# marcopesavento/Super-resolution-3D-Human-Shape-from-a-Single-Low-Resolution-Image

Hardware: AMD Instinct MI355X
Metric: occupancy queries/sec (dense 512^3 reconstruction: encoder + query sweep + 2x marching cubes) (higher is better)
Workload: dtype bf16

## Files before the change

### super-resolution-3d-human-shape-from-a-single-low-resolution-image_amd/csrc/surs_api.cpp

```cpp
#include "surs_common.h"

extern "C" int surs_abi_version(void) { return SURS_ABI_VERSION; }

extern "C" const char *surs_last_error(void) { return surs::err_buf(); }

extern "C" int surs_device_info(int *cu_count, char *arch_out) {
    int dev = 0;
    SURS_HIP_CHECK(hipGetDevice(&dev));
    hipDeviceProp_t prop;
    SURS_HIP_CHECK(hipGetDeviceProperties(&prop, dev));
    if (cu_count) *cu_count = prop.multiProcessorCount;
    if (arch_out) {
        strncpy(arch_out, prop.gcnArchName, 31);
        arch_out[31] = 0;
    }
    return 0;
}

#include <atomic>
#include <cstdlib>
#include <mutex>

namespace {
struct OptionRow {
    const char *name, *env;
    int def;
    char env_first;
    int env_value;
    const char *what;
};
const OptionRow kOptions[surs::OPT_COUNT] = {
    {"split_parts", "SURS_SPLIT", 2, 'b', 3, "operand parts of the fp32-grade GEMMs: 2 (f16 x 2) or 3 (bf16 x 3; env: bf16x3)"},
    {"grid_f32_columns", "SURS_GRID_F32", 1, 'g', 0, "0 (env: gemm): the fp32 sweep on the per-point layer kernels"},
    {"grid_kernel", "SURS_GRID_KERNEL", 0, 0, 0, "reduced-precision column kernel: 0 (default 12), 3, 10, 12"},
    {"grid_f32_kernel", "SURS_GRID_F32_KERNEL", 0, 0, 0, "fp32-grade column kernel: 0 (default 11), 5, 11"},
    {"r_parts", "SURS_R_PARTS", 1, 0, 0, "1: the bf16 sweep's R vectors from one f16 part; 0: the sweep's split"},
    {"grid_f32_passes", "SURS_GRID_F32_PASSES", 2, 0, 0, "passes of the fp32-grade column kernel per batch: 2 (lr, then hr) or 1"},
    {"bicubic_block", "SURS_BICUBIC_BLOCK", 1, 0, 0, "0: bicubic x2 with statistics one output per item (A/B; same bits)"},
    {"mc_emit_reclassify", "SURS_MC_EMIT_RECLASSIFY", 0, 0, 0, "1: marching cubes' emit pass classifies again (tests)"},
    {"point_runs_speculate", "SURS_POINT_RUNS_SPECULATE", 1, 0, 0, "0: surs_query_points_columns reads the run count before it launches"},
    {"conv_trace", "SURS_CONV_TRACE", 0, 0, 0, "diagnostic builds (-DSURS_CONV_TRACE): print the 3x3 kernel's phase stamps"},
    {"v3_trace", "SURS_V3_TRACE", 0, 0, 0, "diagnostic builds (-DSURS_V3_TRACE): print the column kernels' stamps"},
    {"conv_tall_min_wg", "SURS_CONV_TALL_MIN_WG", 256, 0, 0, "workgroups from which a stride-1 3x3 convolution takes the 8-row tile instead of 4 rows (0: never; same bits)"},
    {"conv_wide_min_wg", "SURS_CONV_WIDE_MIN_WG", 512, 0, 0, "workgroups (of 64 channels) from which such a launch takes 8 rows x 64 channels (part of the bits: another order of sums; 0: never)"},
    {"mc_ring", "SURS_MC_RING", 258, 0, 0, "planes of marching cubes' edge -> vertex-id ring = layers per chunk of a one-piece extraction + 1 (66: round 5's)"},
    {"rvec_small", "SURS_RVEC_SMALL", 1, 0, 0, "0: the affine part's GEMM of batches of <= 1024 columns on the 256 x 256-tile kernel (A/B; same bits)"},
};
std::atomic<int> g_option[surs::OPT_COUNT];
std::once_flag g_option_once;
void import_environment() {
    for (int i = 0; i < surs::OPT_COUNT; ++i) {
        const OptionRow &r = kOptions[i];
        int v = r.def;
        if (const char *e = getenv(r.env)) {
            if (r.env_first) v = (e[0] == r.env_first) ? r.env_value : r.def;
            else if (e[0]) v = atoi(e);
        }
        g_option[i].store(v, std::memory_order_relaxed);
    }
}
int find_option(const char *name) {
    if (!name) return -1;
    for (int i = 0; i < surs::OPT_COUNT; ++i)
        if (!strcmp(name, kOptions[i].name) || !strcmp(name, kOptions[i].env)) return i;
    return -1;
}
}

int surs::option(surs::Opt id) {
    std::call_once(g_option_once, import_environment);
    return g_option[id].load(std::memory_order_relaxed);
}

extern "C" int surs_set_option(const char *name, int value) {
    const int i = find_option(name);
    SURS_REQUIRE(i >= 0, "unknown option '%s' (surs_option_name(i) lists them)", name ? name : "(null)");
    std::call_once(g_option_once, import_environment);
    g_option[i].store(value, std::memory_order_relaxed);
    return 0;
}

extern "C" int surs_get_option(const char *name, int *value) {
    const int i = find_option(name);
    SURS_REQUIRE(i >= 0 && value, "unknown option '%s'", name ? name : "(null)");
    *value = surs::option((surs::Opt)i);
    return 0;
}

extern "C" const char *surs_option_name(int index) { return (index >= 0 && index < surs::OPT_COUNT) ? kOptions[index].name : nullptr; }
extern "C" const char *surs_option_help(int index) { return (index >= 0 && index < surs::OPT_COUNT) ? kOptions[index].what : nullptr; }
```

### super-resolution-3d-human-shape-from-a-single-low-resolution-image_amd/csrc/surs_common.h

```cpp
#pragma once
#include <hip/hip_runtime.h>

#include <cstdarg>
#include <cstdio>
#include <cstring>

#include "../../include/surs.h"

namespace surs {

inline char *err_buf() {
    static thread_local char buf[512] = "";
    return buf;
}

inline int fail(int code, const char *fmt, ...) {
    va_list ap;
    va_start(ap, fmt);
    vsnprintf(err_buf(), 512, fmt, ap);
    va_end(ap);
    return code;
}

#define SURS_HIP_CHECK(expr)                                                                     \
    do {                                                                                         \
        hipError_t e_ = (expr);                                                                  \
        if (e_ != hipSuccess)                                                                    \
            return surs::fail(SURS_E_HIP, "%s:%d %s -> %s", __FILE__, __LINE__, #expr, hipGetErrorString(e_)); \
    } while (0)

#define SURS_LAUNCH_CHECK() SURS_HIP_CHECK(hipGetLastError())

#define SURS_REQUIRE(cond, ...)                                   \
    do {                                                          \
        if (!(cond)) return surs::fail(SURS_E_INVALID, __VA_ARGS__); \
    } while (0)

#ifndef SURS_ABL_NO_ISA_PINS
#define SURS_ISA_PIN(v) asm volatile("" : "+v"(v))
#else
#define SURS_ISA_PIN(v) do { } while (0)
#endif

enum Opt {
    OPT_SPLIT_PARTS, OPT_GRID_F32_COLUMNS, OPT_GRID_KERNEL, OPT_GRID_F32_KERNEL, OPT_R_PARTS,
    OPT_GRID_F32_PASSES, OPT_BICUBIC_BLOCK, OPT_MC_EMIT_RECLASSIFY, OPT_POINT_RUNS_SPECULATE, OPT_CONV_TRACE,
    OPT_V3_TRACE, OPT_CONV_TALL_MIN_WG, OPT_CONV_WIDE_MIN_WG, OPT_MC_RING, OPT_RVEC_SMALL, OPT_COUNT
};
int option(Opt id);

inline hipStream_t as_stream(void *s) { return reinterpret_cast<hipStream_t>(s); }

constexpr int ceil_div(long long a, long long b) { return (int)((a + b - 1) / b); }

struct DeviceOnce {
    unsigned long long mask = 0;
    bool first() {
        int dev = 0;
        if (hipGetDevice(&dev) != hipSuccess || dev < 0 || dev >= 64) return true;
        const unsigned long long bit = 1ull << dev;
        const unsigned long long old = __atomic_fetch_or(&mask, bit, __ATOMIC_ACQ_REL);
        return !(old & bit);
    }
};
inline size_t align_up(size_t v, size_t a) { return (v + a - 1) / a * a; }

}
```

### super-resolution-3d-human-shape-from-a-single-low-resolution-image_amd/csrc/surs_gemm.inc

```
__device__ __forceinline__ bool gemm_block_tile(int mblocks, int nblocks, int &mb, int &nb) {
    const unsigned total = (unsigned)mblocks * (unsigned)nblocks, per = gridDim.x >> 3;
    const unsigned logical = (blockIdx.x & 7u) * per + (blockIdx.x >> 3);
    mb = (int)(logical % (unsigned)mblocks);
    nb = (int)(logical / (unsigned)mblocks);
    return logical < total;
}

static inline unsigned gemm_grid(int mblocks, long long nblocks) {
    const long long total = (long long)mblocks * nblocks;
    return (unsigned)(((total + 7) / 8) * 8);
}

struct SplitSeg {
    const unsigned short *base;
    long long part;
    int ktiles;
};

constexpr int G3_STAGES = 3;
constexpr int g3_stage_bytes(int bm, int np_ = 3) { return np_ * ((bm / 32) + 8) * 1024; }
constexpr int g3_lds_bytes(int bm, int np_ = 3) { return G3_STAGES * g3_stage_bytes(bm, np_); }

template <int NP> struct SplitKind;
template <> struct SplitKind<1> {
    typedef _Float16 vec8 __attribute__((ext_vector_type(8)));
    static __device__ __forceinline__ f32x16 mfma(vec8 a, vec8 b, f32x16 c) { return __builtin_amdgcn_mfma_f32_32x32x16_f16(a, b, c, 0, 0, 0); }
    static __device__ __forceinline__ void split(float x, unsigned short (&p)[1]) { p[0] = __builtin_bit_cast(unsigned short, (_Float16)x); }
};
template <> struct SplitKind<3> {
    typedef bf16x8_t vec8;
    static __device__ __forceinline__ f32x16 mfma(vec8 a, vec8 b, f32x16 c) { return __builtin_amdgcn_mfma_f32_32x32x16_bf16(a, b, c, 0, 0, 0); }
    static __device__ __forceinline__ void split(float x, unsigned short (&p)[3]) { split3_bf16(x, p[0], p[1], p[2]); }
};
template <> struct SplitKind<2> {
    typedef _Float16 vec8 __attribute__((ext_vector_type(8)));
    static __device__ __forceinline__ f32x16 mfma(vec8 a, vec8 b, f32x16 c) { return __builtin_amdgcn_mfma_f32_32x32x16_f16(a, b, c, 0, 0, 0); }
    static __device__ __forceinline__ void split(float x, unsigned short (&p)[2]) {
        asm volatile("" : "+v"(x));
        const _Float16 hi = (_Float16)x;
        const _Float16 lo = (_Float16)__builtin_fmaf((float)hi, -1.0f, x);
        p[0] = __builtin_bit_cast(unsigned short, hi);
        p[1] = __builtin_bit_cast(unsigned short, lo);
    }
};

enum { G3_SPLIT = 0, G3_F32 = 1, G3_F32_T = 2 };
template <int NW, int BM, int OUT, int NP = 3>
__global__ __launch_bounds__(NW * 64) void gemm_x3g_kernel(const unsigned short *__restrict__ W3, int M, int Ktot, SplitSeg s1,
                                                           SplitSeg s2, long long np, const float *__restrict__ bias,
                                                           float *__restrict__ Y, long long ldy,
                                                           unsigned short *__restrict__ Ys, long long ys_part, int nblocks) {
    typedef SplitKind<NP> SK;
    typedef typename SK::vec8 vec8;
    constexpr int AP = BM / 32;
    constexpr int TI = AP / 2;
    constexpr int ASZ = NP * AP * 1024;
    constexpr int G3_STAGE = g3_stage_bytes(BM, NP);
    static_assert(NW == 8, "eight waves, 2 x 4");
    static_assert(TI == 4 || TI == 2, "wave tile is 128 or 64 rows");
    static_assert(NP >= 1 && NP <= 3, "one f16 part (not fp32-grade), two f16 parts or three bf16 parts");
    extern __shared__ __attribute__((aligned(16))) unsigned char g3_smem[];
    typedef __attribute__((address_space(3))) unsigned char lds_u8;
    typedef const __attribute__((address_space(1))) void gptr_t;
    const int tid = threadIdx.x, lane = tid & 63, wave = tid >> 6;
    const int wm = wave >> 2, wn = wave & 3;
    const int kh = lane >> 5, li = lane & 31;
    int mb, nb;
    {
        const unsigned mblocks = (unsigned)M / (unsigned)BM, total = mblocks * (unsigned)nblocks, per = gridDim.x >> 3;
        const unsigned logical = (blockIdx.x & 7u) * per + (blockIdx.x >> 3);
        if (logical >= total) return;
        mb = (int)(logical % mblocks);
        nb = (int)(logical / mblocks);
    }
    const long long n0 = (long long)nb * 256;
    const int m0 = mb * BM;
    const int ktiles = s1.ktiles + s2.ktiles;
    const size_t per_part = (size_t)Ktot * M;
    lds_u8 *smem = (lds_u8 *)g3_smem;
    const unsigned lds0 = (unsigned)(size_t)smem;

    f32x16 acc[TI][2];
#pragma unroll
    for (int i = 0; i < TI; ++i)
#pragma unroll
        for (int j = 0; j < 2; ++j)
#pragma unroll
            for (int r = 0; r < 16; ++r) acc[i][j][r] = 0.0f;

    const int piece = wave & 7;
    const bool both = BM == 256 || wave < 4;
    const int nd = both ? 2 * NP : NP;
    const unsigned short *wsrc = W3 + ((size_t)(m0 + 32 * piece)) * 16 + lane * 8;
    auto issue1 = [&](int kt, int d) {
        const int p = both ? d >> 1 : d;
        const bool points = both ? (d & 1) : (NW == 8 || wave >= 8);
        lds_u8 *stage = smem + (kt % G3_STAGES) * G3_STAGE + piece * 1024;
        if (!points) {
            const unsigned short *wk = wsrc + (size_t)kt * M * 16 + p * per_part;
            __builtin_amdgcn_global_load_lds((gptr_t *)wk, (__attribute__((address_space(3))) void *)(stage + p * (AP * 1024)), 16, 0, 0);
        } else {
            const bool first = kt < s1.ktiles;
            const unsigned short *xb = first ? s1.base : s2.base;
            const long long xpart = first ? s1.part : s2.part;
            const int k = first ? kt : kt - s1.ktiles;
            const unsigned short *xsrc = xb + ((long long)k * np + n0 + 32 * piece) * 16 + (li * 16 + kh * 8) + p * xpart;
            __builtin_amdgcn_global_load_lds((gptr_t *)xsrc, (__attribute__((address_space(3))) void *)(stage + ASZ + p * 8192), 16, 0, 0);
        }
    };
    auto issue = [&](int kt) {
        for (int d = 0; d < nd; ++d) issue1(kt, d);
    };

    issue(0);
    if (ktiles > 1) issue(1);
    const unsigned a_off = lds0 + (unsigned)(wm * TI * 1024 + lane * 16);
    const unsigned b_off = lds0 + (unsigned)ASZ + (unsigned)(wn * 2048 + lane * 16);
    vec8 a[TI][NP], b[2][NP];
    auto mm = [&](int pa, int pb) {
#pragma unroll
        for (int i = 0; i < TI; ++i)
#pragma unroll
            for (int j = 0; j < 2; ++j) {
                if constexpr (OUT == G3_F32_T) acc[i][j] = SK::mfma(b[j][pb], a[i][pa], acc[i][j]);
                else acc[i][j] = SK::mfma(a[i][pa], b[j][pb], acc[i][j]);
            }
    };
#ifdef SURS_G3_NO_LDS
#define G3_RD(dst, addr, off) asm volatile("" : "=v"(dst) : "v"(addr) : "memory")
// ... 24 lines not shown
            if constexpr (NP == 3 && TI == 2) { if (t == 0) G3_WAIT2(8, 2, 0); else if (t == 1) G3_WAIT2(4, 1, 1); else G3_WAIT2(0, 0, 2); }
            if constexpr (NP == 2 && TI == 4) { if (t == 0) G3_WAIT4(6, 1, 0); else G3_WAIT4(0, 0, 1); }
            if constexpr (NP == 2 && TI == 2) { if (t == 0) G3_WAIT2(4, 1, 0); else G3_WAIT2(0, 0, 1); }
            if constexpr (NP == 1 && TI == 4) G3_WAIT4(0, 0, 0);
            if constexpr (NP == 1 && TI == 2) G3_WAIT2(0, 0, 0);
            mm(NP - 1 - t, t);
            __builtin_amdgcn_sched_barrier(0);
            if (more)
                for (int d = t * nd / NP; d < (t + 1) * nd / NP; ++d) issue1(kt + 2, d);
        }
    };
    auto phase2 = [&](int kt) {
        if constexpr (NP == 3) {
            mm(1, 0);
            mm(0, 1);
        }
        if constexpr (NP > 1) mm(0, 0);
        __builtin_amdgcn_sched_barrier(0);
    };
    auto step_barrier = [&](int kt) {
#ifdef SURS_G3_NO_DMA
        asm volatile("s_waitcnt vmcnt(0)\n\ts_barrier" ::: "memory");
#else
        if (kt + 1 < ktiles) {
            if (nd == 6) asm volatile("s_waitcnt vmcnt(6)\n\ts_barrier" ::: "memory");
            else if (nd == 4) asm volatile("s_waitcnt vmcnt(4)\n\ts_barrier" ::: "memory");
            else if (nd == 3) asm volatile("s_waitcnt vmcnt(3)\n\ts_barrier" ::: "memory");
            else if (nd == 1) asm volatile("s_waitcnt vmcnt(1)\n\ts_barrier" ::: "memory");
            else asm volatile("s_waitcnt vmcnt(2)\n\ts_barrier" ::: "memory");
        } else
            asm volatile("s_waitcnt vmcnt(0)\n\ts_barrier" ::: "memory");
#endif
    };
    if (((wave >> 2) & 1) == 0) {
        for (int kt = 0; kt < ktiles; ++kt) {
            step_barrier(kt);
            phase1(kt);
            phase2(kt);
        }
    } else {
        step_barrier(0);
        phase1(0);
        for (int kt = 1; kt < ktiles; ++kt) {
            step_barrier(kt);
            phase2(kt - 1);
            phase1(kt);
        }
        phase2(ktiles - 1);
    }

#undef G3_RD
#undef G3_WAIT4
#undef G3_WAIT2
#pragma unroll
    for (int i = 0; i < TI; ++i)
#pragma unroll
        for (int j = 0; j < 2; ++j) {
            const long long n = n0 + wn * 64 + j * 32 + li;
            const int mrow = m0 + wm * (TI * 32) + i * 32;
            if constexpr (OUT == G3_F32_T) {
                const long long nb0 = n0 + wn * 64 + j * 32 + 4 * kh;
                const float bm = bias[mrow + li];
#pragma unroll
                for (int g = 0; g < 4; ++g)
#pragma unroll
                    for (int r = 0; r < 4; ++r) Y[(nb0 + 8 * g + r) * ldy + mrow + li] = acc[i][j][4 * g + r] + bm;
                continue;
            }
            float v[16];
#pragma unroll
            for (int g = 0; g < 4; ++g)
#pragma unroll
                for (int r = 0; r < 4; ++r) {
                    float t = acc[i][j][4 * g + r] + bias[mrow + 8 * g + 4 * kh + r];
                    v[4 * g + r] = t > 0.0f ? t : 0.01f * t;
                }
            if constexpr (OUT == G3_F32) {
#pragma unroll
                for (int g = 0; g < 4; ++g)
#pragma unroll
                    for (int r = 0; r < 4; ++r) Y[(long long)(mrow + 8 * g + 4 * kh + r) * ldy + n] = v[4 * g + r];
            } else
#pragma unroll
            for (int q = 0; q < 2; ++q) {
                unsigned e[NP][2], o[NP][2];
#pragma unroll
                for (int d = 0; d < 2; ++d) {
                    unsigned short x0[NP], x1[NP], y0[NP], y1[NP];
                    SK::split(v[8 * q + 2 * d], x0);
                    SK::split(v[8 * q + 2 * d + 1], x1);
                    SK::split(v[8 * q + 4 + 2 * d], y0);
                    SK::split(v[8 * q + 4 + 2 * d + 1], y1);
#pragma unroll
                    for (int p = 0; p < NP; ++p) {
                        e[p][d] = (unsigned)x0[p] | ((unsigned)x1[p] << 16);
                        o[p][d] = (unsigned)y0[p] | ((unsigned)y1[p] << 16);
                    }
                }
                unsigned short *dst = Ys + ((long long)((mrow >> 4) + q) * np + n) * 16 + kh * 8;
#pragma unroll
                for (int p = 0; p < NP; ++p) {
                    const auto t0 = __builtin_amdgcn_permlane32_swap(e[p][0], o[p][0], false, false);
                    const auto t1 = __builtin_amdgcn_permlane32_swap(e[p][1], o[p][1], false, false);
                    u32x4 w = {t0[0], t1[0], t0[1], t1[1]};
                    *reinterpret_cast<u32x4 *>(dst + p * ys_part) = w;
                }
// ... 82 lines not shown
```

### super-resolution-3d-human-shape-from-a-single-low-resolution-image_amd/csrc/surs_query.hip

```cpp
#include <hip/hip_runtime.h>

#include <cstdlib>
#include <map>
#include <mutex>
#include <type_traits>
#include <utility>
#include <vector>

#include "surs_common.h"
#include "surs_mlp_generic.h"
#include "surs_mlp_layout.h"

namespace surs {

typedef float f32x16 __attribute__((ext_vector_type(16)));
typedef float f32x4 __attribute__((ext_vector_type(4)));
typedef unsigned u32x4 __attribute__((ext_vector_type(4)));
typedef unsigned u32x2 __attribute__((ext_vector_type(2)));
typedef float f32x2 __attribute__((ext_vector_type(2)));

struct PointSource {
    int mode;
    const float *pts;
    const long long *idx;
// ... 290 lines not shown
    unsigned short *Fs, *Y0s, *Y1s, *Y2s;
    long long np;
};

static size_t fp32_ws_bytes(long long np) {
    return (size_t)np * ((C0PAD + D4 + 1) * sizeof(float) + (size_t)(C0PAD + D1 + D2 + D3) * 6) + 4096;
}

static Fp32Workspace carve_fp32(void *ws, long long np) {
    Fp32Workspace w;
    float *p = (float *)ws;
    w.np = np;
    w.F = p; p += (size_t)C0PAD * np;
    w.Y3 = p; p += (size_t)D4 * np;
    w.mask = p; p += np;
    unsigned short *q = (unsigned short *)p;
    w.Fs = q; q += (size_t)3 * C0PAD * np;
    w.Y0s = q; q += (size_t)3 * D1 * np;
    w.Y1s = q; q += (size_t)3 * D2 * np;
    w.Y2s = q;
    return w;
}

static int g_split_override = 0;
static thread_local int t_split_call = 0;
static int split_parts() {
    const int v = option(OPT_SPLIT_PARTS) == 3 ? 3 : 2;
    return t_split_call > 1 ? t_split_call : (g_split_override ? g_split_override : v);
}

template <int NP, int... More, class F> static void with_parts(int parts, F &&f) {
    if constexpr (sizeof...(More) == 0) f(std::integral_constant<int, NP>());
    else if (parts == NP) f(std::integral_constant<int, NP>());
    else with_parts<More...>(parts, f);
}

static int g3_set_attributes() {
    static DeviceOnce attr;
    if (attr.first()) {
        SURS_HIP_CHECK(hipFuncSetAttribute((const void *)gemm_x3g_kernel<8, 256, G3_SPLIT, 2>, hipFuncAttributeMaxDynamicSharedMemorySize, g3_lds_bytes(256, 2)));
        SURS_HIP_CHECK(hipFuncSetAttribute((const void *)gemm_x3g_kernel<8, 256, G3_F32, 2>, hipFuncAttributeMaxDynamicSharedMemorySize, g3_lds_bytes(256, 2)));
        SURS_HIP_CHECK(hipFuncSetAttribute((const void *)gemm_x3g_kernel<8, 128, G3_F32, 2>, hipFuncAttributeMaxDynamicSharedMemorySize, g3_lds_bytes(128, 2)));
        SURS_HIP_CHECK(hipFuncSetAttribute((const void *)gemm_x3g_kernel<8, 128, G3_F32_T, 2>, hipFuncAttributeMaxDynamicSharedMemorySize, g3_lds_bytes(128, 2)));
        SURS_HIP_CHECK(hipFuncSetAttribute((const void *)gemm_x3g_kernel<8, 256, G3_SPLIT>, hipFuncAttributeMaxDynamicSharedMemorySize, g3_lds_bytes(256)));
        SURS_HIP_CHECK(hipFuncSetAttribute((const void *)gemm_x3g_kernel<8, 256, G3_F32>, hipFuncAttributeMaxDynamicSharedMemorySize, g3_lds_bytes(256)));
        SURS_HIP_CHECK(hipFuncSetAttribute((const void *)gemm_x3g_kernel<8, 128, G3_F32>, hipFuncAttributeMaxDynamicSharedMemorySize, g3_lds_bytes(128)));
        SURS_HIP_CHECK(hipFuncSetAttribute((const void *)gemm_x3g_kernel<8, 128, G3_F32_T>, hipFuncAttributeMaxDynamicSharedMemorySize, g3_lds_bytes(128)));
        SURS_HIP_CHECK(hipFuncSetAttribute((const void *)gemm_x3g_kernel<8, 256, G3_F32_T, 2>, hipFuncAttributeMaxDynamicSharedMemorySize, g3_lds_bytes(256, 2)));
        SURS_HIP_CHECK(hipFuncSetAttribute((const void *)gemm_x3g_kernel<8, 256, G3_F32_T>, hipFuncAttributeMaxDynamicSharedMemorySize, g3_lds_bytes(256)));
        SURS_HIP_CHECK(hipFuncSetAttribute((const void *)gemm_x3g_kernel<8, 256, G3_F32_T, 1>, hipFuncAttributeMaxDynamicSharedMemorySize, g3_lds_bytes(256, 1)));
        SURS_HIP_CHECK(hipFuncSetAttribute((const void *)gemm_x3g_kernel<8, 256, G3_SPLIT, 1>, hipFuncAttributeMaxDynamicSharedMemorySize, g3_lds_bytes(256, 1)));
        SURS_HIP_CHECK(hipFuncSetAttribute((const void *)gemm_x3g_kernel<8, 256, G3_F32, 1>, hipFuncAttributeMaxDynamicSharedMemorySize, g3_lds_bytes(256, 1)));
        SURS_HIP_CHECK(hipFuncSetAttribute((const void *)gemm_x3g_kernel<8, 128, G3_F32, 1>, hipFuncAttributeMaxDynamicSharedMemorySize, g3_lds_bytes(128, 1)));
    }
    return 0;
}

static int launch_layer(hipStream_t st, int parts, int out, const void *W, int M, SplitSeg s1, SplitSeg s2, long long np, long long n,
                        const float *bias, float *Y, unsigned short *Ys) {
    SURS_REQUIRE(parts >= 1 && parts <= 3, "layer kernel: 1, 2 or 3 operand parts");
    SURS_REQUIRE(np % 256 == 0 && n % 256 == 0 && n <= np, "the layer kernel needs 256-point tiles");
    SURS_REQUIRE(M % 256 == 0 || (out != G3_SPLIT && M % 128 == 0), "layer kernel rows: a multiple of 256 (of 128 for an fp32 output)");
    SURS_REQUIRE(M % 256 == 0 || out != G3_F32_T || parts > 1, "no one-part layer kernel for a transposed output of 128-row tiles");
    int rc = g3_set_attributes();
    if (rc) return rc;
    const int K = 16 * (s1.ktiles + s2.ktiles), nb = (int)(n / 256);
    const long long ldy = out == G3_F32_T ? M : np;
    with_parts<1, 2, 3>(parts, [&](auto NP) {
        auto go = [&](auto BM, auto OUT) {
            hipLaunchKernelGGL((gemm_x3g_kernel<8, BM, OUT, NP>), dim3(gemm_grid(M / BM, nb)), dim3(512), g3_lds_bytes(BM, NP), st,
                               (const unsigned short *)W, M, K, s1, s2, np, bias, Y, ldy, Ys, (long long)M * np, nb);
        };
        using C256 = std::integral_constant<int, 256>;
        using C128 = std::integral_constant<int, 128>;
        if (out == G3_SPLIT) go(C256(), std::integral_constant<int, G3_SPLIT>());
        else if (out == G3_F32) {
            if (M % 256 == 0) go(C256(), std::integral_constant<int, G3_F32>());
            else go(C128(), std::integral_constant<int, G3_F32>());
        } else if (M % 256 == 0) go(C256(), std::integral_constant<int, G3_F32_T>());
        else if constexpr (NP > 1) go(C128(), std::integral_constant<int, G3_F32_T>());
    });
    SURS_LAUNCH_CHECK();
    return 0;
}

static int run_points_fp32(hipStream_t st, const PointSource &src, long long n, const float *feat_lr, int hl, int wl,
                           const float *feat_hr, int hh, int wh, const char *blob, const MlpBlobHeader &h,
                           const Fp32Workspace &w, float *pred_hr, float *pred_lr, float *logit_hr, float *logit_lr,
                           int parts = 0, const float *p_lr_in = nullptr, bool lr_only = false) {
    const long long np = w.np;
    if (parts == 0) parts = t_split_call == 1 ? 1 : split_parts();
    const long long fs_part = (long long)C0PAD * np;
    with_parts<1, 2, 3>(parts, [&](auto NP) {
        hipLaunchKernelGGL(gather_kernel<NP>, dim3((unsigned)ceil_div(n, 64)), dim3(256), 0, st, src, n, feat_lr, hl, wl, feat_hr,
                           hh, wh, w.F, np, w.mask, (float *)nullptr, w.Fs, fs_part);
    });
    SURS_LAUNCH_CHECK();
    if (p_lr_in) {
        with_parts<1, 2, 3>(parts, [&](auto NP) {
            hipLaunchKernelGGL(patch_plr_kernel<NP>, dim3((unsigned)ceil_div(n, 256)), dim3(256), 0, st, p_lr_in, np, n,
                               w.F + (size_t)(C_G + 1) * np, w.Fs, fs_part);
        });
        SURS_LAUNCH_CHECK();
    }
    const SplitSeg none = {nullptr, 0, 0}, f = {w.Fs, fs_part, C0PAD / 16}, y0 = {w.Y0s, (long long)D1 * np, D1 / 16},
                   y1 = {w.Y1s, (long long)D2 * np, D2 / 16}, y2 = {w.Y2s, (long long)D3 * np, D3 / 16};
    for (int m = p_lr_in ? 1 : 0; m < (lr_only ? 1 : 2); ++m) {
        auto W = [&](int l) { return (const void *)(blob + (parts <= 2 ? h.wt2[m][l] : h.wt3[m][l])); };
        auto BI = [&](int l) { return (const float *)(blob + h.bias[m][l]); };
        int rc;
        if ((rc = launch_layer(st, parts, G3_SPLIT, W(0), D1, f, none, np, np, BI(0), nullptr, w.Y0s))) return rc;
        if ((rc = launch_layer(st, parts, G3_SPLIT, W(1), D2, y0, none, np, np, BI(1), nullptr, w.Y1s))) return rc;
        if ((rc = launch_layer(st, parts, G3_SPLIT, W(2), D3, y1, f, np, np, BI(2), nullptr, w.Y2s))) return rc;
        if ((rc = launch_layer(st, parts, G3_F32, W(3), D4, y2, f, np, np, BI(3), w.Y3, nullptr))) return rc;
        with_parts<1, 2, 3>(parts, [&](auto NP) {
            hipLaunchKernelGGL(mlp_last_kernel<NP>, dim3((unsigned)ceil_div(n, 256)), dim3(256), 0, st,
                               (const float *)(blob + h.w4[m]), w.Y3, w.F, np, n, w.mask, m == 0 ? pred_lr : pred_hr,
                               m == 0 ? logit_lr : logit_hr, m == 0 ? w.F + (size_t)(C_G + 1) * np : (float *)nullptr,
                               m == 0 ? w.Fs : (unsigned short *)nullptr, fs_part);
        });
        SURS_LAUNCH_CHECK();
    }
    return 0;
}

template <int DT> struct HalfT;
template <> struct HalfT<SURS_BF16> {
    typedef __bf16 elem;
    typedef __bf16 vec8 __attribute__((ext_vector_type(8)));
    typedef __bf16 vec2 __attribute__((ext_vector_type(2)));
    static __device__ __forceinline__ f32x16 mfma(vec8 a, vec8 b, f32x16 c) {
        return __builtin_amdgcn_mfma_f32_32x32x16_bf16(a, b, c, 0, 0, 0);
    }
// ... 421 lines not shown
    for (auto &e : g_prof.ev) SURS_HIP_CHECK(hipEventSynchronize(e.second));
    unsigned long long v = 0;
    for (auto &k : g_prof.kstat) {
        unsigned long long one = 0;
        SURS_HIP_CHECK(hipMemcpy(&one, k.second, sizeof(one), hipMemcpyDeviceToHost));
        v += one;
    }
    if (tile_mlps) *tile_mlps = g_prof.tiles;
    if (ksteps) *ksteps = (double)v;
    return 0;
}

static const long long GRID_BATCH = 65536;
#ifndef SURS_COL_BATCH
#define SURS_COL_BATCH 32768
#endif
static const long long COL_BATCH = SURS_COL_BATCH;

static size_t col_base_bytes(long long ncb) {
    return (size_t)ncb * (C0PAD + CC_PAD + 1) * sizeof(float) + (size_t)ncb * C0PAD * 6 + 4096;
}
static size_t col_v7_image_bytes(long long ncb) { return (size_t)ncb * 5 * D1 * 6; }
static size_t col_v7_bytes(long long ncb) { return col_v7_image_bytes(ncb) + (size_t)ncb * 5 * D2 * 4 + D2 * 4 + 256; }
static size_t col_ws_bytes(long long ncb) { return col_base_bytes(ncb) + col_v7_bytes(ncb); }

extern "C" size_t surs_query_grid_workspace_bytes(int ry, int rz, int dtype) {
    (void)ry; (void)rz;
    const size_t col = col_ws_bytes(COL_BATCH);
    if (dtype == SURS_F32 || dtype == SURS_F32_GEMM) {
        const size_t gen = fp32_ws_bytes(GRID_BATCH);
        return gen > col ? gen : col;
    }
    return col;
}

static bool grid_f32_use_columns() { return option(OPT_GRID_F32_COLUMNS) != 0; }

static int grid_set_attributes() {
    static DeviceOnce attr;
    if (!attr.first()) return 0;
    SURS_HIP_CHECK(hipFuncSetAttribute((const void *)grid_mlp_kernel_v3<SURS_BF16>, hipFuncAttributeMaxDynamicSharedMemorySize, GRID3_LDS_BYTES));
    SURS_HIP_CHECK(hipFuncSetAttribute((const void *)grid_mlp_kernel_v3<SURS_F16>, hipFuncAttributeMaxDynamicSharedMemorySize, GRID3_LDS_BYTES));
    SURS_HIP_CHECK(hipFuncSetAttribute((const void *)grid_mlp_kernel_v5, hipFuncAttributeMaxDynamicSharedMemorySize, GRID5_LDS_BYTES));
    SURS_HIP_CHECK(hipFuncSetAttribute((const void *)grid_mlp_kernel_v11, hipFuncAttributeMaxDynamicSharedMemorySize, GRID11_LDS_BYTES));
    SURS_HIP_CHECK(hipFuncSetAttribute((const void *)grid_mlp_kernel_v10<SURS_BF16>, hipFuncAttributeMaxDynamicSharedMemorySize, GRID10_LDS_BYTES));
    SURS_HIP_CHECK(hipFuncSetAttribute((const void *)grid_mlp_kernel_v10<SURS_F16>, hipFuncAttributeMaxDynamicSharedMemorySize, GRID10_LDS_BYTES));
    SURS_HIP_CHECK(hipFuncSetAttribute((const void *)grid_mlp_kernel_v12<SURS_BF16>, hipFuncAttributeMaxDynamicSharedMemorySize, GRID12_LDS_BYTES));
    SURS_HIP_CHECK(hipFuncSetAttribute((const void *)grid_mlp_kernel_v12<SURS_F16>, hipFuncAttributeMaxDynamicSharedMemorySize, GRID12_LDS_BYTES));
    return 0;
}

static int column_constants(hipStream_t st, const PointSource &src, long long nc, long long ncp, const float *feat_lr, int hl, int wl,
                            const float *feat_hr, int hh, int wh, const char *blob, const MlpBlobHeader &h, float *F, float *CC,
                            float *cmask) {
    const int parts = split_parts();
    unsigned short *Fs = (unsigned short *)(cmask + COL_BATCH);
    const long long fs_part = (long long)C0PAD * COL_BATCH;
    const dim3 gg((unsigned)ceil_div(nc, 64), nc <= 4096 ? 5u : 1u);
    with_parts<2, 3>(parts, [&](auto NP) {
        hipLaunchKernelGGL(gather_kernel<NP>, gg, dim3(256), 0, st, src, nc, feat_lr, hl, wl, feat_hr, hh, wh, F, COL_BATCH, cmask,
                           (float *)nullptr, Fs, fs_part);
    });
    SURS_LAUNCH_CHECK();
    const SplitSeg f = {Fs, fs_part, C_G / 16}, none = {nullptr, 0, 0};
    return launch_layer(st, parts, G3_F32_T, blob + (parts == 2 ? h.wc2 : h.wc3), CC_PAD, f, none, COL_BATCH, ncp,
                        (const float *)(blob + h.bc), CC, nullptr);
}

__global__ __launch_bounds__(256) void probe_count_kernel(const float *__restrict__ cc, const float *__restrict__ zvec, int rz, int tile,
                                                          double z0, double dz, float c22, float c23, float zmul, float zdiv, float zmid,
                                                          unsigned long long *__restrict__ out) {
    const int tid = threadIdx.x;
    const float *row = cc + (size_t)blockIdx.x * CC_PAD;
    const f32x4 al = *reinterpret_cast<const f32x4 *>(row + CC_A0_LR + 4 * tid), ah = *reinterpret_cast<const f32x4 *>(row + CC_A0_HR + 4 * tid);
    const f32x4 zl = *reinterpret_cast<const f32x4 *>(zvec + ZV_W0Z_LR + 4 * tid), zh = *reinterpret_cast<const f32x4 *>(zvec + ZV_W0Z_HR + 4 * tid);
    const f32x4 ph = *reinterpret_cast<const f32x4 *>(zvec + ZV_W0P_HR + 4 * tid);
    auto zf_of = [&](int k) {
        const double zt = dz * (double)k;
        const float zw = (float)(zt + z0);
        const float Z = c23 + c22 * zw;
        return Z * zmul / zdiv;
    };
    unsigned nl = 0, nh = 0;
    for (int k0 = 0; k0 < rz; k0 += tile) {
        const float e0 = zf_of(k0), e1 = zf_of(k0 + tile - 1);
        const float zlo = fminf(e0, e1), zhi = fmaxf(e0, e1);
#pragma unroll
        for (int i = 0; i < 4; ++i) {
            {
                const float xm = fmaf(zmid, zl[i], al[i]);
                const float t0 = zl[i] * zlo, t1 = zl[i] * zhi;
                const float mn = al[i] + fminf(t0, t1), mx = al[i] + fmaxf(t0, t1);
                nl += ((xm > 0.0f) ? (mn > 0.0f) : (mx <= 0.0f)) ? 0u : 1u;
            }
            {
                const float xm = fmaf(0.5f, ph[i], fmaf(zmid, zh[i], ah[i]));
                const float t0 = zh[i] * zlo, t1 = zh[i] * zhi;
                const float mn = ah[i] + fminf(t0, t1) + fminf(0.0f, ph[i]), mx = ah[i] + fmaxf(t0, t1) + fmaxf(0.0f, ph[i]);
                nh += ((xm > 0.0f) ? (mn > 0.0f) : (mx <= 0.0f)) ? 0u : 1u;
            }
        }
    }
#pragma unroll
    for (int d = 32; d >= 1; d >>= 1) {
        nl += __shfl_xor(nl, d);
        nh += __shfl_xor(nh, d);
    }
    if ((tid & 63) == 0) {
        atomicAdd(out, (unsigned long long)nl);
        atomicAdd(out + 1, (unsigned long long)nh);
    }
}

static int query_grid_impl(int i0, int i1, int ry, int rz, const double *mat, const float *calib, float zmul,
                           float zdiv, const float *feat_lr, int hl, int wl, const float *feat_hr, int hh, int wh,
                           const void *mlp_blob, int dtype, void *workspace, size_t workspace_bytes, float *vol_hr,
                           float *vol_lr, int kernel_call, void *stream);

extern "C" int surs_query_grid_opt(int i0, int i1, int ry, int rz, const double *mat, const float *calib, float zmul,
                                   float zdiv, const float *feat_lr, int hl, int wl, const float *feat_hr, int hh, int wh,
                                   const void *mlp_blob, int dtype, void *workspace, size_t workspace_bytes, float *vol_hr,
                                   float *vol_lr, const SursGridOptions *opt, void *stream) {
    int kernel = 0, parts = 0;
    if (opt) {
        kernel = opt->kernel;
        parts = opt->operand_parts;
        SURS_REQUIRE(grid_kernel_known(kernel), "SursGridOptions.kernel: 0, 3, 10, 12 (reduced precision), 5, 11 (fp32-grade)");
        SURS_REQUIRE(parts == 0 || parts == 2 || parts == 3, "SursGridOptions.operand_parts: 0, 2 or 3");
    }
    const int saved = t_split_call;
    if (parts) t_split_call = parts;
    const int rc = query_grid_impl(i0, i1, ry, rz, mat, calib, zmul, zdiv, feat_lr, hl, wl, feat_hr, hh, wh, mlp_blob, dtype, workspace,
                                   workspace_bytes, vol_hr, vol_lr, kernel, stream);
    t_split_call = saved;
    return rc;
}

extern "C" int surs_query_grid(int i0, int i1, int ry, int rz, const double *mat, const float *calib, float zmul,
                               float zdiv, const float *feat_lr, int hl, int wl, const float *feat_hr, int hh, int wh,
                               const void *mlp_blob, int dtype, void *workspace, size_t workspace_bytes, float *vol_hr,
                               float *vol_lr, void *stream) {
    return query_grid_impl(i0, i1, ry, rz, mat, calib, zmul, zdiv, feat_lr, hl, wl, feat_hr, hh, wh, mlp_blob, dtype, workspace,
                           workspace_bytes, vol_hr, vol_lr, 0, stream);
}

namespace {
struct ColumnSweep {
    hipStream_t st;
    const char *blob;
    MlpBlobHeader h;
    int dtype;
    int kver, kver32;
    bool restated;
    const float *feat_lr; int hl, wl;
    const float *feat_hr; int hh, wh;
    const double *mat; const float *calib; float zmul, zdiv;
    void *workspace;
    int cus;
    int kmid;
    const int *run_colstart = nullptr;
    const float *run_z = nullptr;
    const int *run_tiles = nullptr;
    const unsigned *run_ntiles = nullptr;
    long long run_ntiles_host = 0;
};
}

static void resolve_column_kernels(int kernel_call, int &kver, int &kver32) {
    const int ve = option(OPT_GRID_KERNEL), ve32 = option(OPT_GRID_F32_KERNEL);
    const int kver_env = (ve == 3 || ve == 10 || ve == 12) ? ve : SURS_DEFAULT_GRID_KERNEL;
    const int kver32_env = (ve32 == 5 || ve32 == 11) ? ve32 : SURS_DEFAULT_GRID_F32_KERNEL;
    const auto is32 = [](int v) { return v == 5 || v == 11; };
    kver = kver_env;
    kver32 = kver32_env;
    if (g_grid_kernel_override) (is32(g_grid_kernel_override) ? kver32 : kver) = g_grid_kernel_override;
    if (kernel_call) (is32(kernel_call) ? kver32 : kver) = kernel_call;
}

static int device_cus() {
    int dev = 0;
    hipDeviceProp_t prop;
    if (hipGetDevice(&dev) == hipSuccess && hipGetDeviceProperties(&prop, dev) == hipSuccess) return prop.multiProcessorCount;
    return 256;
}

static int run_column_batch(const ColumnSweep &cs, const PointSource &src, long long nc, int items, int zstride,
                            const int *kcount, const unsigned short *klist, float *vol_hr, float *vol_lr, bool trace_this) {
    hipStream_t st = cs.st;
    const char *blob = cs.blob;
    const MlpBlobHeader &h = cs.h;
    const int dtype = cs.dtype, kver = cs.kver, kver32 = cs.kver32;
    const bool restated = cs.restated;
    const double *mat = cs.mat;
    const float *calib = cs.calib;
    void *workspace = cs.workspace;
    float *F = (float *)workspace;
    float *CC = F + (size_t)C0PAD * COL_BATCH;
    float *cmask = CC + (size_t)CC_PAD * COL_BATCH;
    int rc = 0;
    const long long ncp = (long long)ceil_div(nc, 256) * 256;
    const int parts = split_parts();
    if ((rc = column_constants(st, src, nc, ncp, cs.feat_lr, cs.hl, cs.wl, cs.feat_hr, cs.hh, cs.wh, blob, h, F, CC, cmask))) return rc;
    GridArgs a;
    a.cc = CC;
    a.colmask = cmask;
    a.zvec = (const float *)(blob + h.zvec);
    a.core = blob + h.core;
    a.corex = blob + h.corex;
    a.b1frag = blob + h.b1frag;
    a.b1_inv_scale = 1.0f / (dtype == SURS_F16 ? B1FRAG_SCALE_F16 : B1FRAG_SCALE_BF16);
    a.w1t = blob + h.w1t;
    a.w1tx = blob + h.w1tx;
    a.rvec_lr = a.rvec_hr = nullptr;
    a.rld_lr = a.rld_hr = 0;
    a.colctr = nullptr;
    a.phase = 0;
    a.zmid = 0.0f;
    a.zstride = zstride;
    a.kcount = kcount;
    a.klist = klist;
    a.ovf_count = nullptr;
    a.ovf_list = nullptr;
    a.tile_list = cs.run_tiles;
    a.tile_count = cs.run_ntiles;
    a.colstart = cs.run_colstart;
    a.zpts = cs.run_z;
    if (restated) {
        char *v7 = (char *)workspace + col_base_bytes(COL_BATCH);
        unsigned short *g_lr = (unsigned short *)v7, *g_hr = g_lr + (size_t)COL_BATCH * 2 * D1 * 3;
        float *r_lr = (float *)(v7 + col_v7_image_bytes(COL_BATCH)), *r_hr = r_lr + (size_t)COL_BATCH * 2 * D2;
        float *zero_bias = r_hr + (size_t)COL_BATCH * 3 * D2;
        SURS_HIP_CHECK(hipMemsetAsync(zero_bias, 0, D2 * 4 + 256, st));
        a.colctr = (unsigned *)(zero_bias + D2);
        {
            const float zw = cs.run_z ? 0.0f : (float)(mat[10] * (double)cs.kmid + mat[11]);
            a.zmid = (calib[11] + calib[10] * zw) * cs.zmul / cs.zdiv;
        }
        const long long part_lr = 2LL * ncp * D1, part_hr = 3LL * ncp * D1;
        const dim3 pg((unsigned)(ncp / 4));
        const int r_parts_env = option(OPT_R_PARTS);
        const int rparts = (dtype == SURS_BF16 && r_parts_env == 1) ? 1 : parts;
        with_parts<1, 2, 3>(rparts, [&](auto NP) {
            hipLaunchKernelGGL(colsum_prepare_kernel<NP>, pg, dim3(256), 0, st, CC, (const float *)(blob + h.zvec), (int)ncp, a.zmid,
                               g_lr, part_lr, g_hr, part_hr);
        });
        SURS_LAUNCH_CHECK();
        if (ncp <= 1024 && option(OPT_RVEC_SMALL)) {
            RvecSmallArgs ra;
            for (int m = 0; m < 2; ++m) {
                const int nvec = m ? 3 : 2;
                ra.w[m] = (const unsigned short *)(blob + (rparts == 3 ? h.wt3[m][1] : h.wt2[m][1]));
                ra.g[m] = m ? g_hr : g_lr;
                ra.g_part[m] = m ? part_hr : part_lr;
                ra.npm[m] = (long long)nvec * ncp;
                ra.r[m] = m ? r_hr : r_lr;
            }
            ra.wgs0 = (int)(ra.npm[0] / 64) * 4;
            const unsigned wgs = (unsigned)(ra.wgs0 + (ra.npm[1] / 64) * 4);
            with_parts<1, 2, 3>(rparts, [&](auto NP) { hipLaunchKernelGGL(rvec_small_kernel<NP>, dim3(wgs), dim3(256), 0, st, ra); });
            SURS_LAUNCH_CHECK();
        } else {
            const SplitSeg none = {nullptr, 0, 0};
            for (int m = 0; m < 2; ++m) {
                const long long npm = (m ? 3LL : 2LL) * ncp;
                const SplitSeg g = {m ? g_hr : g_lr, m ? part_hr : part_lr, D1 / 16};
                if ((rc = launch_layer(st, rparts, G3_F32_T, blob + (rparts == 3 ? h.wt3[m][1] : h.wt2[m][1]), D2, g, none, npm, npm,
                                       zero_bias, m ? r_hr : r_lr, nullptr)))
                    return rc;
            }
        }
        a.rvec_lr = r_lr;
        a.rvec_hr = r_hr;
        a.rld_lr = a.rld_hr = 0;
    }
    a.vol_hr = vol_hr;
    a.vol_lr = vol_lr;
    a.ncols = (int)nc;
    a.rz = items;
    a.z0 = mat ? mat[11] : 0.0;
    a.dz = mat ? mat[10] : 0.0;
    a.c22 = calib[10];
    a.c23 = calib[11];
    a.zmul = cs.zmul;
    a.zdiv = cs.zdiv;
    const long long nwork = cs.run_tiles ? cs.run_ntiles_host : nc;
    const unsigned grid = (unsigned)((nwork < cs.cus) ? nwork : cs.cus);
    hipEvent_t e0 = nullptr, e1 = nullptr;
    bool prof;
    a.kstat = nullptr;
    {
        std::lock_guard<std::mutex> lock(g_prof.mu);
        prof = g_prof.on && !kcount;
        if (prof && restated) {
            int dev = 0;
            SURS_HIP_CHECK(hipGetDevice(&dev));
            unsigned long long *&ctr = g_prof.kstat[dev];
            if (!ctr) {
                SURS_HIP_CHECK(hipMalloc((void **)&ctr, sizeof(unsigned long long)));
                SURS_HIP_CHECK(hipMemset(ctr, 0, sizeof(unsigned long long)));
// ... 750 lines not shown
```

Baseline: 1.112 billion.

## Fuse colsum g-image preparation into the column-constant GEMM epilogue

Adds a templated epilogue to the column-constant GEMM. It computes the gated, split g-vectors for the lr and hr rows directly from the accumulators, stages them in LDS and writes them to the g-image buffers. It also clears the column counters. This removes the separate colsum_prepare_kernel launch and its reread of CC, and the zero-bias memset now runs once per context instead of every batch. The risks are extra LDS staging and register pressure in the GEMM epilogue, plus a new launch-bounds hint that could change occupancy.

```diff
diff --git a/super-resolution-3d-human-shape-from-a-single-low-resolution-image_amd/csrc/surs_api.cpp b/super-resolution-3d-human-shape-from-a-single-low-resolution-image_amd/csrc/surs_api.cpp
--- a/super-resolution-3d-human-shape-from-a-single-low-resolution-image_amd/csrc/surs_api.cpp
+++ b/super-resolution-3d-human-shape-from-a-single-low-resolution-image_amd/csrc/surs_api.cpp
@@ -45,6 +45,7 @@
     {"conv_wide_min_wg", "SURS_CONV_WIDE_MIN_WG", 512, 0, 0, "workgroups (of 64 channels) from which such a launch takes 8 rows x 64 channels (part of the bits: another order of sums; 0: never)"},
     {"mc_ring", "SURS_MC_RING", 258, 0, 0, "planes of marching cubes' edge -> vertex-id ring = layers per chunk of a one-piece extraction + 1 (66: round 5's)"},
     {"rvec_small", "SURS_RVEC_SMALL", 1, 0, 0, "0: the affine part's GEMM of batches of <= 1024 columns on the 256 x 256-tile kernel (A/B; same bits)"},
+    {"colsum_fused", "SURS_COLSUM_FUSED", 1, 0, 0, "0: the g-scaled vectors of a restated sweep from colsum_prepare_kernel instead of the column-constant GEMM's epilogue (A/B; same bits)"},
 };
 std::atomic<int> g_option[surs::OPT_COUNT];
 std::once_flag g_option_once;
diff --git a/super-resolution-3d-human-shape-from-a-single-low-resolution-image_amd/csrc/surs_common.h b/super-resolution-3d-human-shape-from-a-single-low-resolution-image_amd/csrc/surs_common.h
--- a/super-resolution-3d-human-shape-from-a-single-low-resolution-image_amd/csrc/surs_common.h
+++ b/super-resolution-3d-human-shape-from-a-single-low-resolution-image_amd/csrc/surs_common.h
@@ -45,7 +45,7 @@
 enum Opt {
     OPT_SPLIT_PARTS, OPT_GRID_F32_COLUMNS, OPT_GRID_KERNEL, OPT_GRID_F32_KERNEL, OPT_R_PARTS,
     OPT_GRID_F32_PASSES, OPT_BICUBIC_BLOCK, OPT_MC_EMIT_RECLASSIFY, OPT_POINT_RUNS_SPECULATE, OPT_CONV_TRACE,
-    OPT_V3_TRACE, OPT_CONV_TALL_MIN_WG, OPT_CONV_WIDE_MIN_WG, OPT_MC_RING, OPT_RVEC_SMALL, OPT_COUNT
+    OPT_V3_TRACE, OPT_CONV_TALL_MIN_WG, OPT_CONV_WIDE_MIN_WG, OPT_MC_RING, OPT_RVEC_SMALL, OPT_COLSUM_FUSED, OPT_COUNT
 };
 int option(Opt id);
 
diff --git a/super-resolution-3d-human-shape-from-a-single-low-resolution-image_amd/csrc/surs_gemm.inc b/super-resolution-3d-human-shape-from-a-single-low-resolution-image_amd/csrc/surs_gemm.inc
--- a/super-resolution-3d-human-shape-from-a-single-low-resolution-image_amd/csrc/surs_gemm.inc
+++ b/super-resolution-3d-human-shape-from-a-single-low-resolution-image_amd/csrc/surs_gemm.inc
@@ -45,11 +45,23 @@
 };
 
 enum { G3_SPLIT = 0, G3_F32 = 1, G3_F32_T = 2 };
-template <int NW, int BM, int OUT, int NP = 3>
-__global__ __launch_bounds__(NW * 64) void gemm_x3g_kernel(const unsigned short *__restrict__ W3, int M, int Ktot, SplitSeg s1,
+struct G3Gimg {
+    const float *zvec;
+    unsigned short *g_lr, *g_hr;
+    long long part_lr, part_hr;
+    long long ncp;
+    float zmid;
+    unsigned *clear;
+};
+constexpr int G3_GSTAGE = 9216;
+template <int NW, int BM, int OUT, int NP = 3, int GP = 0>
+__global__ __launch_bounds__(NW * 64, (GP > 0 && NP == 2) ? 4 : 1) void gemm_x3g_kernel(const unsigned short *__restrict__ W3, int M, int Ktot, SplitSeg s1,
                                                            SplitSeg s2, long long np, const float *__restrict__ bias,
                                                            float *__restrict__ Y, long long ldy,
-                                                           unsigned short *__restrict__ Ys, long long ys_part, int nblocks) {
+                                                           unsigned short *__restrict__ Ys, long long ys_part, int nblocks,
+                                                           G3Gimg gi) {
+    static_assert(GP == 0 || (OUT == G3_F32_T && BM == 128 && NP >= 2 && CC_A0_LR == 0 && CC_A0_HR == D1 && D1 % BM == 0),
+                  "the g-image epilogue belongs to the column-constant GEMM: whole 128-row tiles of a0, >= 72 KB of LDS");
     typedef SplitKind<NP> SK;
     typedef typename SK::vec8 vec8;
     constexpr int AP = BM / 32;
@@ -75,6 +87,9 @@
     }
     const long long n0 = (long long)nb * 256;
     const int m0 = mb * BM;
+    if constexpr (GP > 0) {
+        if (blockIdx.x == 0 && tid < 3) gi.clear[tid] = 0u;
+    }
     const int ktiles = s1.ktiles + s2.ktiles;
     const size_t per_part = (size_t)Ktot * M;
     lds_u8 *smem = (lds_u8 *)g3_smem;
@@ -205,6 +220,88 @@
 #undef G3_RD
 #undef G3_WAIT4
 #undef G3_WAIT2
+    [[maybe_unused]] auto gimage = [&](auto NVc, const float (&v)[16], int mrow, long long col0) {
+        constexpr int NV = decltype(NVc)::value;
+        constexpr int GQ = GP > 0 ? GP : 1;
+        constexpr int CS = 32 * NV * 32 + 8 * 32 + 64;
+        static_assert(2 * CS <= G3_GSTAGE && CS % 16 == 0, "two channel groups per wave and sub-tile");
+        typedef SplitKind<GQ> GK;
+        const int ch0 = mrow - (NV == 3 ? CC_A0_HR : CC_A0_LR);
+        int ln = lane;
+        asm volatile("" : "+v"(ln));
+        const int li = ln & 31, kh = ln >> 5;
+        const float wz = gi.zvec[(NV == 3 ? ZV_W0Z_HR : ZV_W0Z_LR) + ch0 + li];
+        const float wp = NV == 3 ? gi.zvec[ZV_W0P_HR + ch0 + li] : 0.0f;
+        unsigned char *stg = g3_smem + wave * G3_GSTAGE;
+        unsigned char *wr = stg + (li >> 4) * CS + kh * (4 * NV * 32 + 32) + (li & 15) * 2;
+        unsigned short *img = NV == 3 ? gi.g_hr : gi.g_lr;
+        const long long part = NV == 3 ? gi.part_hr : gi.part_lr, npm = NV * gi.ncp;
+#pragma unroll
+        for (int q = 0; q < GQ; ++q) {
+#pragma unroll
+            for (int g = 0; g < 4; ++g)
+#pragma unroll
+                for (int r = 0; r < 4; ++r) {
+                    float a0 = v[4 * g + r];
+                    asm volatile("" : "+v"(a0));
+                    const float x = NV == 3 ? fmaf(0.5f, wp, fmaf(gi.zmid, wz, a0)) : fmaf(gi.zmid, wz, a0);
+                    const float gg = x > 0.0f ? 1.0f : 0.01f;
+                    float val[3] = {gg * a0, gg * wz, gg * wp};
+#pragma unroll
+                    for (int vv = 0; vv < NV; ++vv) {
+                        unsigned short p[GQ];
+                        SURS_ISA_PIN(val[vv]);
+                        GK::split(val[vv], p);
+                        *reinterpret_cast<unsigned short *>(wr + g * (8 * NV * 32 + 64) + r * (NV * 32) + vv * 32) = p[q];
+                    }
+                }
+            __builtin_amdgcn_fence(__ATOMIC_RELEASE, "wavefront");
+            __builtin_amdgcn_wave_barrier();
+            __builtin_amdgcn_sched_barrier(0);
+            __builtin_amdgcn_fence(__ATOMIC_ACQUIRE, "wavefront");
+#pragma unroll
+            for (int c = 0; c < 2; ++c)
+#pragma unroll
+                for (int t = 0; t < NV; ++t) {
+                    const int idx = ln + 64 * t, pt = idx / (2 * NV);
+                    const u32x4 w = *reinterpret_cast<const u32x4 *>(stg + c * CS + idx * 16 + (pt >> 2) * 32);
+                    *reinterpret_cast<u32x4 *>(img + q * part + ((long long)((ch0 >> 4) + c) * npm + NV * col0) * 16 + idx * 8) = w;
+                }
+            __builtin_amdgcn_fence(__ATOMIC_RELEASE, "wavefront");
+            __builtin_amdgcn_wave_barrier();
+            __builtin_amdgcn_sched_barrier(0);
+            __builtin_amdgcn_fence(__ATOMIC_ACQUIRE, "wavefront");
+        }
+    };
+    if constexpr (GP > 0) {
+        auto tile = [&](auto NVc) {
+            constexpr int NV = decltype(NVc)::value;
+            if constexpr (NV > 0) __syncthreads();
+#pragma unroll
+            for (int i = 0; i < TI; ++i)
+#pragma unroll
+                for (int j = 0; j < 2; ++j) {
+                    __builtin_amdgcn_sched_barrier(0);
+                    const int mrow = m0 + wm * (TI * 32) + i * 32;
+                    const long long nb0 = n0 + wn * 64 + j * 32 + 4 * kh;
+                    const float bm = bias[mrow + li];
+                    long long ld = ldy;
+                    asm volatile("" : "+s"(ld));
+                    float v[16];
+#pragma unroll
+                    for (int k = 0; k < 16; ++k) v[k] = acc[i][j][k] + bm;
+#pragma unroll
+                    for (int g = 0; g < 4; ++g)
+#pragma unroll
+                        for (int r = 0; r < 4; ++r) Y[(nb0 + 8 * g + r) * ld + mrow + li] = v[4 * g + r];
+                    if constexpr (NV > 0) gimage(NVc, v, mrow, n0 + wn * 64 + j * 32);
+                }
+        };
+        if (m0 < CC_A0_HR) tile(std::integral_constant<int, 2>());
+        else if (m0 < CC_A0_HR + D1) tile(std::integral_constant<int, 3>());
+        else tile(std::integral_constant<int, 0>());
+        return;
+    }
 #pragma unroll
     for (int i = 0; i < TI; ++i)
 #pragma unroll
diff --git a/super-resolution-3d-human-shape-from-a-single-low-resolution-image_amd/csrc/surs_query.hip b/super-resolution-3d-human-shape-from-a-single-low-resolution-image_amd/csrc/surs_query.hip
--- a/super-resolution-3d-human-shape-from-a-single-low-resolution-image_amd/csrc/surs_query.hip
+++ b/super-resolution-3d-human-shape-from-a-single-low-resolution-image_amd/csrc/surs_query.hip
@@ -366,16 +366,22 @@
         SURS_HIP_CHECK(hipFuncSetAttribute((const void *)gemm_x3g_kernel<8, 256, G3_SPLIT, 1>, hipFuncAttributeMaxDynamicSharedMemorySize, g3_lds_bytes(256, 1)));
         SURS_HIP_CHECK(hipFuncSetAttribute((const void *)gemm_x3g_kernel<8, 256, G3_F32, 1>, hipFuncAttributeMaxDynamicSharedMemorySize, g3_lds_bytes(256, 1)));
         SURS_HIP_CHECK(hipFuncSetAttribute((const void *)gemm_x3g_kernel<8, 128, G3_F32, 1>, hipFuncAttributeMaxDynamicSharedMemorySize, g3_lds_bytes(128, 1)));
+        SURS_HIP_CHECK(hipFuncSetAttribute((const void *)gemm_x3g_kernel<8, 128, G3_F32_T, 2, 1>, hipFuncAttributeMaxDynamicSharedMemorySize, g3_lds_bytes(128, 2)));
+        SURS_HIP_CHECK(hipFuncSetAttribute((const void *)gemm_x3g_kernel<8, 128, G3_F32_T, 2, 2>, hipFuncAttributeMaxDynamicSharedMemorySize, g3_lds_bytes(128, 2)));
+        SURS_HIP_CHECK(hipFuncSetAttribute((const void *)gemm_x3g_kernel<8, 128, G3_F32_T, 3, 1>, hipFuncAttributeMaxDynamicSharedMemorySize, g3_lds_bytes(128, 3)));
+        SURS_HIP_CHECK(hipFuncSetAttribute((const void *)gemm_x3g_kernel<8, 128, G3_F32_T, 3, 3>, hipFuncAttributeMaxDynamicSharedMemorySize, g3_lds_bytes(128, 3)));
     }
     return 0;
 }
 
 static int launch_layer(hipStream_t st, int parts, int out, const void *W, int M, SplitSeg s1, SplitSeg s2, long long np, long long n,
-                        const float *bias, float *Y, unsigned short *Ys) {
+                        const float *bias, float *Y, unsigned short *Ys, const G3Gimg *gimg = nullptr, int gparts = 0) {
     SURS_REQUIRE(parts >= 1 && parts <= 3, "layer kernel: 1, 2 or 3 operand parts");
     SURS_REQUIRE(np % 256 == 0 && n % 256 == 0 && n <= np, "the layer kernel needs 256-point tiles");
     SURS_REQUIRE(M % 256 == 0 || (out != G3_SPLIT && M % 128 == 0), "layer kernel rows: a multiple of 256 (of 128 for an fp32 output)");
     SURS_REQUIRE(M % 256 == 0 || out != G3_F32_T || parts > 1, "no one-part layer kernel for a transposed output of 128-row tiles");
+    SURS_REQUIRE(!gimg || (out == G3_F32_T && M == CC_PAD && parts > 1 && (gparts == 1 || gparts == parts) && gimg->ncp == n),
+                 "the g-image epilogue belongs to the column-constant GEMM");
     int rc = g3_set_attributes();
     if (rc) return rc;
     const int K = 16 * (s1.ktiles + s2.ktiles), nb = (int)(n / 256);
@@ -383,7 +389,7 @@
     with_parts<1, 2, 3>(parts, [&](auto NP) {
         auto go = [&](auto BM, auto OUT) {
             hipLaunchKernelGGL((gemm_x3g_kernel<8, BM, OUT, NP>), dim3(gemm_grid(M / BM, nb)), dim3(512), g3_lds_bytes(BM, NP), st,
-                               (const unsigned short *)W, M, K, s1, s2, np, bias, Y, ldy, Ys, (long long)M * np, nb);
+                               (const unsigned short *)W, M, K, s1, s2, np, bias, Y, ldy, Ys, (long long)M * np, nb, G3Gimg());
         };
         using C256 = std::integral_constant<int, 256>;
         using C128 = std::integral_constant<int, 128>;
@@ -392,7 +398,17 @@
             if (M % 256 == 0) go(C256(), std::integral_constant<int, G3_F32>());
             else go(C128(), std::integral_constant<int, G3_F32>());
         } else if (M % 256 == 0) go(C256(), std::integral_constant<int, G3_F32_T>());
-        else if constexpr (NP > 1) go(C128(), std::integral_constant<int, G3_F32_T>());
+        else if constexpr (NP > 1) {
+            if (!gimg) go(C128(), std::integral_constant<int, G3_F32_T>());
+            else {
+                auto gog = [&](auto GP) {
+                    hipLaunchKernelGGL((gemm_x3g_kernel<8, 128, G3_F32_T, NP, GP>), dim3(gemm_grid(M / 128, nb)), dim3(512), g3_lds_bytes(128, NP),
+                                       st, (const unsigned short *)W, M, K, s1, s2, np, bias, Y, ldy, Ys, (long long)M * np, nb, *gimg);
+                };
+                if (gparts == 1) gog(std::integral_constant<int, 1>());
+                else gog(NP);
+            }
+        }
     });
     SURS_LAUNCH_CHECK();
     return 0;
@@ -920,7 +936,7 @@
 
 static int column_constants(hipStream_t st, const PointSource &src, long long nc, long long ncp, const float *feat_lr, int hl, int wl,
                             const float *feat_hr, int hh, int wh, const char *blob, const MlpBlobHeader &h, float *F, float *CC,
-                            float *cmask) {
+                            float *cmask, const G3Gimg *gimg = nullptr, int gparts = 0) {
     const int parts = split_parts();
     unsigned short *Fs = (unsigned short *)(cmask + COL_BATCH);
     const long long fs_part = (long long)C0PAD * COL_BATCH;
@@ -932,7 +948,7 @@
     SURS_LAUNCH_CHECK();
     const SplitSeg f = {Fs, fs_part, C_G / 16}, none = {nullptr, 0, 0};
     return launch_layer(st, parts, G3_F32_T, blob + (parts == 2 ? h.wc2 : h.wc3), CC_PAD, f, none, COL_BATCH, ncp,
-                        (const float *)(blob + h.bc), CC, nullptr);
+                        (const float *)(blob + h.bc), CC, nullptr, gimg, gparts);
 }
 
 __global__ __launch_bounds__(256) void probe_count_kernel(const float *__restrict__ cc, const float *__restrict__ zvec, int rz, int tile,
@@ -1031,6 +1047,7 @@
     const int *run_tiles = nullptr;
     const unsigned *run_ntiles = nullptr;
     long long run_ntiles_host = 0;
+    mutable bool zero_bias_written = false;
 };
 }
 
@@ -1068,7 +1085,29 @@
     int rc = 0;
     const long long ncp = (long long)ceil_div(nc, 256) * 256;
     const int parts = split_parts();
-    if ((rc = column_constants(st, src, nc, ncp, cs.feat_lr, cs.hl, cs.wl, cs.feat_hr, cs.hh, cs.wh, blob, h, F, CC, cmask))) return rc;
+    const bool fused = restated && option(OPT_COLSUM_FUSED) != 0;
+    char *v7 = (char *)workspace + col_base_bytes(COL_BATCH);
+    unsigned short *g_lr = (unsigned short *)v7, *g_hr = g_lr + (size_t)COL_BATCH * 2 * D1 * 3;
+    float *r_lr = (float *)(v7 + col_v7_image_bytes(COL_BATCH)), *r_hr = r_lr + (size_t)COL_BATCH * 2 * D2;
+    float *zero_bias = r_hr + (size_t)COL_BATCH * 3 * D2;
+    unsigned *colctr = (unsigned *)(zero_bias + D2);
+    const long long part_lr = 2LL * ncp * D1, part_hr = 3LL * ncp * D1;
+    const int rparts = (dtype == SURS_BF16 && option(OPT_R_PARTS) == 1) ? 1 : parts;
+    float zmid = 0.0f;
+    if (restated) {
+        const float zw = cs.run_z ? 0.0f : (float)(mat[10] * (double)cs.kmid + mat[11]);
+        zmid = (calib[11] + calib[10] * zw) * cs.zmul / cs.zdiv;
+    }
+    if (fused) {
+        if (!cs.zero_bias_written) {
+            SURS_HIP_CHECK(hipMemsetAsync(zero_bias, 0, D2 * 4 + 256, st));
+            cs.zero_bias_written = true;
+        }
+        const G3Gimg gimg = {(const float *)(blob + h.zvec), g_lr, g_hr, part_lr, part_hr, ncp, zmid, colctr};
+        rc = column_constants(st, src, nc, ncp, cs.feat_lr, cs.hl, cs.wl, cs.feat_hr, cs.hh, cs.wh, blob, h, F, CC, cmask, &gimg, rparts);
+    } else
+        rc = column_constants(st, src, nc, ncp, cs.feat_lr, cs.hl, cs.wl, cs.feat_hr, cs.hh, cs.wh, blob, h, F, CC, cmask);
+    if (rc) return rc;
     GridArgs a;
     a.cc = CC;
     a.colmask = cmask;
@@ -1094,25 +1133,17 @@
     a.colstart = cs.run_colstart;
     a.zpts = cs.run_z;
     if (restated) {
-        char *v7 = (char *)workspace + col_base_bytes(COL_BATCH);
-        unsigned short *g_lr = (unsigned short *)v7, *g_hr = g_lr + (size_t)COL_BATCH * 2 * D1 * 3;
-        float *r_lr = (float *)(v7 + col_v7_image_bytes(COL_BATCH)), *r_hr = r_lr + (size_t)COL_BATCH * 2 * D2;
-        float *zero_bias = r_hr + (size_t)COL_BATCH * 3 * D2;
-        SURS_HIP_CHECK(hipMemsetAsync(zero_bias, 0, D2 * 4 + 256, st));
-        a.colctr = (unsigned *)(zero_bias + D2);
-        {
-            const float zw = cs.run_z ? 0.0f : (float)(mat[10] * (double)cs.kmid + mat[11]);
-            a.zmid = (calib[11] + calib[10] * zw) * cs.zmul / cs.zdiv;
-        }
-        const long long part_lr = 2LL * ncp * D1, part_hr = 3LL * ncp * D1;
-        const dim3 pg((unsigned)(ncp / 4));
-        const int r_parts_env = option(OPT_R_PARTS);
-        const int rparts = (dtype == SURS_BF16 && r_parts_env == 1) ? 1 : parts;
-        with_parts<1, 2, 3>(rparts, [&](auto NP) {
-            hipLaunchKernelGGL(colsum_prepare_kernel<NP>, pg, dim3(256), 0, st, CC, (const float *)(blob + h.zvec), (int)ncp, a.zmid,
-                               g_lr, part_lr, g_hr, part_hr);
-        });
-        SURS_LAUNCH_CHECK();
+        a.colctr = colctr;
+        a.zmid = zmid;
+        if (!fused) {
+            SURS_HIP_CHECK(hipMemsetAsync(zero_bias, 0, D2 * 4 + 256, st));
+            const dim3 pg((unsigned)(ncp / 4));
+            with_parts<1, 2, 3>(rparts, [&](auto NP) {
+                hipLaunchKernelGGL(colsum_prepare_kernel<NP>, pg, dim3(256), 0, st, CC, (const float *)(blob + h.zvec), (int)ncp, a.zmid,
+                                   g_lr, part_lr, g_hr, part_hr);
+            });
+            SURS_LAUNCH_CHECK();
+        }
         if (ncp <= 1024 && option(OPT_RVEC_SMALL)) {
             RvecSmallArgs ra;
             for (int m = 0; m < 2; ++m) {
```

After: 1.122 billion (median of 6 runs). No clear change (+0.9%).
